# sandyz1000/face-landmark-detector

Hardware: AMD Instinct MI355X
Metric: faces/sec (whole node), 256x256 batch inference: fused preprocess + FCN-8 forward + softmax + top-4 landmark decode + similarity/alignment warp (higher is better)
Workload: dtype f32; 1 GPU; BASELINE configs[1]: batch=64/GPU 256x256x3 uint8 crops, fcn_8(68) vanilla encoder fp32, random-init weights (seed 2), decode top-4 thresh 0, align to 256x256; global_batch=64, parallelism=dp1

## Files before the change

### face-landmark-detector_amd/build.py

```python
from __future__ import annotations

import concurrent.futures
import hashlib
import os
import shutil
import subprocess
import sys

HERE = os.path.dirname(os.path.abspath(__file__))
ROOT = os.path.dirname(HERE)
CSRC = os.path.join(HERE, "csrc")
INCLUDE = os.path.join(ROOT, "include")
OBJ_DIR = os.path.join(HERE, "csrc", "build")
LIB_PATH = os.path.join(HERE, "libflm_hip.so")

SOURCES = [
    "flm_api.hip",
    "flm_pack.hip",
    "flm_enc1.hip",
    "flm_igemm.hip",
    "flm_igemm_bf16.hip",
    "flm_conv3_halo.hip",
    "flm_score1x1.hip",
    "flm_tail_bf16.hip",
    "flm_convt.hip",
    "flm_up3_wreg.hip",
    "flm_decode.hip",
    "flm_decode_stats.hip",
    "flm_cand.hip",
    "flm_misc.hip",
    "flm_frames.hip",
    "flm_warp_fmt.hip",
    "flm_frames_nv12.hip",
    "flm_mesh.hip",
    "flm_track.hip",
    "flm_track_assoc.hip",
    "flm_quality.hip",
    "flm_track_exit.hip",
    "flm_track_views.hip",
    "flm_pose.hip",
    "flm_annotate.hip",
    "flm_flow.hip",
    "flm_mobile.hip",
]
FLAGS = ["--offload-arch=gfx950", "-O3", "-fPIC", "-std=c++17", "-ffp-contract=off",
         "-Wall", "-Wno-unused-function", "-I", INCLUDE, "-I", CSRC]


FILE_FLAGS = {"flm_enc1.hip": ["-mllvm", "-amdgpu-mfma-vgpr-form"]}


def _hipcc() -> str:
    for c in (shutil.which("hipcc"), "/opt/rocm/bin/hipcc"):
        if c and os.path.exists(c):
            return c
    raise RuntimeError("hipcc not found: the HIP extension cannot be built")


def _stamp(paths) -> str:
    h = hashlib.sha256()
    h.update(" ".join(FLAGS).encode())
    h.update(repr(sorted(FILE_FLAGS.items())).encode())
    for p in sorted(paths):
        with open(p, "rb") as f:
            h.update(p.encode())
            h.update(f.read())
    return h.hexdigest()


def build(force: bool = False, verbose: bool = True, extra_flags=()) -> str:
    os.makedirs(OBJ_DIR, exist_ok=True)
    headers = [os.path.join(CSRC, f) for f in os.listdir(CSRC) if f.endswith(".h")] + \
              [os.path.join(INCLUDE, f) for f in os.listdir(INCLUDE) if f.endswith(".h")]
    srcs = [os.path.join(CSRC, s) for s in SOURCES]
    stamp = _stamp(srcs + headers) + " ".join(extra_flags)
    stamp_file = os.path.join(OBJ_DIR, "stamp.txt")
    if not force and os.path.exists(LIB_PATH) and os.path.exists(stamp_file) and open(stamp_file).read() == stamp:
        return LIB_PATH
    hipcc = _hipcc()

    def compile_one(src):
        obj = os.path.join(OBJ_DIR, os.path.basename(src) + ".o")
        cmd = [hipcc, *FLAGS, *FILE_FLAGS.get(os.path.basename(src), []), *extra_flags, "-c", src, "-o", obj]
        r = subprocess.run(cmd, capture_output=True, text=True)
        if r.returncode != 0:
            raise RuntimeError("hipcc failed on %s:\n%s\n%s" % (src, r.stdout, r.stderr))
        if verbose and r.stderr.strip():
            sys.stderr.write(r.stderr)
        return obj

    with concurrent.futures.ThreadPoolExecutor(max_workers=min(8, len(srcs))) as ex:
        objs = list(ex.map(compile_one, srcs))
    cmd = [hipcc, "--offload-arch=gfx950", "-shared", "-fPIC", "-o", LIB_PATH, *objs]
    r = subprocess.run(cmd, capture_output=True, text=True)
    if r.returncode != 0:
        raise RuntimeError("link failed:\n%s\n%s" % (r.stdout, r.stderr))
    with open(stamp_file, "w") as f:
        f.write(stamp)
    if verbose:
        print("built", LIB_PATH)
    return LIB_PATH


if __name__ == "__main__":
    build(force="--force" in sys.argv)
```

### face-landmark-detector_amd/csrc/flm_api.hip

```cpp
#include <cmath>
#include <cstdarg>
#include <cstdio>
#include <cstring>

#include "flm_annotate_dev.h"
#include "flm_common.h"

namespace flm {

static thread_local char g_err[512] = "";

void set_error(const char* fmt, ...) {
  va_list ap;
  va_start(ap, fmt);
  vsnprintf(g_err, sizeof(g_err), fmt, ap);
  va_end(ap);
}

int hip_fail(hipError_t e, const char* what) {
  set_error("HIP error %d (%s) at %s", (int)e, hipGetErrorString(e), what);
  return FLM_ERR_HIP;
}

struct Knob {
  const char* key;
  std::atomic<int> value;
  bool (*valid)(int);
  const char* domain;
};
static Knob g_knobs[] = {
    {"bf16_big_tiles", {1}, nullptr, nullptr},
    {"bf16_lds_dma", {1}, nullptr, nullptr},
    {"bf16_mfma16", {1}, nullptr, nullptr},
    {"bf16_halo_mfma16", {1}, nullptr, nullptr},
    {"f32_two_level", {1}, nullptr, nullptr},
    {"f32_lean_tile", {1}, nullptr, nullptr},
    {"bf16_group_n", {0}, [](int v) { return v >= 0 && v <= 32 && !(v & (v - 1)); }, "0 or a power of two <= 32"},
    {"bf16_conv3_halo", {1}, nullptr, nullptr},
    {"bf16_score1x1", {1}, nullptr, nullptr},
    {"bf16_fused_tail", {1}, nullptr, nullptr},
    {"decode_lds_dma", {1}, nullptr, nullptr},
    {"posmajor_order", {1}, nullptr, nullptr},
    {"warp_rows", {1}, [](int v) { return v == 0 || v == 1 || v == 4; }, "0, 1 or 4"},
    {"up3_cand8", {1}, [](int v) { return v >= 0 && v <= 7; }, "in [0,7]"},
    {"up3_cand8_rows", {0}, [](int v) { return v >= 0 && v <= 8 && !(v & (v - 1)); }, "0, 1, 2, 4 or 8"},
    {"up3_wreg", {0}, [](int v) { return v == 0 || v == 1; }, "0 or 1"},
    {"f32_fc6_rows", {0}, [](int v) { return v == 0 || v == 64 || v == 128; }, "0, 64 or 128"},
};
static_assert(sizeof(g_knobs) / sizeof(g_knobs[0]) == KNOB_COUNT, "one row per KnobId");
int tuning(KnobId id) { return g_knobs[id].value.load(std::memory_order_relaxed); }
static Knob* find_knob(const char* who, const char* key) {
  for (Knob& k : g_knobs)
    if (!strcmp(k.key, key)) return &k;
  set_error("%s: unknown key '%s'", who, key);
  return nullptr;
}

struct ProfRec {
  const char* name;
  hipEvent_t a, b;
};
static ProfRec* g_prof = nullptr;
static int g_prof_cap = 0, g_prof_n = 0;
static char g_prof_filter[32] = "";

struct ProfScope {
  hipStream_t s;
  ProfRec* r;
  ProfScope(hipStream_t st, const char* name) : s(st), r(nullptr) {
    if (name && g_prof && g_prof_n < g_prof_cap && (!g_prof_filter[0] || !strcmp(g_prof_filter, name))) {
      r = &g_prof[g_prof_n++];
      r->name = name;
      (void)hipEventRecord(r->a, s);
    }
  }
  ~ProfScope() {
    if (r) (void)hipEventRecord(r->b, s);
  }
};

struct CandOpts {
  int enable, sub, cap_div;
};
static bool resolve_opts(const flm_forward_opts* o, CandOpts* c) {
  c->enable = 1;
  c->sub = 0;
  c->cap_div = 1;
  if (!o) return true;
  if (o->struct_size < sizeof(flm_forward_opts)) {
    set_error("flm_forward_opts: struct_size %u is smaller than this library's %zu (initialise with flm_forward_opts_init)",
              o->struct_size, sizeof(flm_forward_opts));
    return false;
  }
  if (o->candidate_sub_phases < 0 || o->candidate_sub_phases > 16 || o->candidate_cap_div < 1) {
    set_error("flm_forward_opts: candidate_sub_phases must be in [0,16] and candidate_cap_div >= 1");
    return false;
  }
  c->enable = o->landmark_candidates != 0;
  c->sub = o->candidate_sub_phases;
  c->cap_div = o->candidate_cap_div;
  return true;
}
static int cand_sub_for(const CandOpts& c, int n_points, bool bf16) {
  if (c.sub > 0) return c.sub;
  return n_points <= 8 ? (bf16 ? 4 : 2) : (n_points <= 15 ? 6 : 8);
}
static bool landmark_candidates_enabled(const CandOpts& c, const ConvTGeom& g, int fcn32, int decode_mode, int n_points,
                                        int oh, int ow) {
  return c.enable && !fcn32 && decode_mode == FLM_DECODE_TOPN && n_points >= 1 && n_points <= 32 &&
         convt_candidates_supported(g) && (long long)oh * ow < (1 << 17);
}

struct EncNames {
  char s[kMaxEnc][8];
  EncNames() {
    for (int i = 0; i < kMaxEnc; ++i) snprintf(s[i], sizeof(s[i]), "enc%d", i + 1);
  }
};

static size_t take(size_t& cur, size_t bytes) {
  size_t o = cur;
  cur = align_up(cur + bytes, 256);
  return o;
}

Fcn8Ws fcn8_ws_layout(int n, int h, int w, int C, int dtype, int out_mode, int decode_mode, int n_points,
                      int arch, const flm_forward_opts* opts) {
  Fcn8Ws W;
  CandOpts co;
  if (!resolve_opts(opts, &co)) {
    W = Fcn8Ws();
    W.total = 0;
    return W;
  }
  const ConvTGeom g = convt_geom(C, dtype);
  const ArchSpec A = arch_spec(arch);
  const size_t es = dtype == FLM_BF16 ? 2 : 4;
  size_t cur = 0;
  int hs[kMaxEnc], wsz[kMaxEnc];
  enc_dims(A, h, w, hs, wsz);
  for (int i = 0; i < A.n_enc; ++i) W.act[i] = take(cur, es * (size_t)n * hs[i] * wsz[i] * A.enc[i].cout);
  for (int k = 0; k < 5; ++k) W.f[k] = W.act[A.f_idx[k]];
  const int h5 = h / 32, w5 = w / 32, h4 = h / 16, w4 = w / 16, h3 = h / 8, w3 = w / 8;
  W.fc6 = take(cur, es * (size_t)n * h5 * w5 * kFc);
  W.fc7 = take(cur, es * (size_t)n * h5 * w5 * kFc);
  W.score5 = take(cur, sizeof(float) * (size_t)n * h5 * w5 * g.Cp);
  W.fuse4 = take(cur, sizeof(float) * (size_t)n * h4 * w4 * g.Cp);
  W.seg = take(cur, sizeof(float) * (size_t)n * h3 * w3 * g.Cp);
  W.splitk_bytes = sizeof(float) * 8 * (size_t)n * h5 * w5 * g.Cp;
  {
    const size_t rows = (size_t)n * h5 * w5 < 256 ? (size_t)n * h5 * w5 : 256;
    const size_t fc_bytes = sizeof(float) * 8 * rows * kFc;
    if (fc_bytes > W.splitk_bytes) W.splitk_bytes = fc_bytes;
  }
  if (n <= 4) {
    const size_t enc3_bytes = sizeof(float) * 4 * (size_t)4 * (h / 4) * (w / 4) * 256;
    if (enc3_bytes > W.splitk_bytes) W.splitk_bytes = enc3_bytes;
  }
  W.splitk = take(cur, W.splitk_bytes);
  W.oh = h + (A.fcn32 ? 32 : 8);
  W.ow = w + (A.fcn32 ? 32 : 8);
  W.probs = SIZE_MAX;
  W.decode = SIZE_MAX;
  W.sub = W.tau = W.cand = W.cand_cnt = SIZE_MAX;
  W.cand_cap = W.cand_sub = 0;
  const int stats = out_mode == FLM_OUT_LANDMARKS_STATS;
  if (out_mode == FLM_OUT_LANDMARKS || stats) {
    W.probs = take(cur, sizeof(float) * (size_t)n * W.oh * W.ow * C);
    W.decode = take(cur, decode_ws_bytes(n, W.oh, W.ow, C, decode_mode, n_points, stats));
    if (landmark_candidates_enabled(co, g, A.fcn32, decode_mode, n_points, W.oh, W.ow)) {
      W.cand_sub = cand_sub_for(co, n_points, g.bf16 != 0);
      W.sub = take(cur, sizeof(unsigned) * (size_t)n * convt_sample_slots(g, h3, w3, W.cand_sub) * 16 * g.MT);
      W.tau = take(cur, sizeof(float) * (size_t)n * C);
      W.cand_cap = (int)align_up((size_t)C * 64 * n_points * 4 / co.cap_div, 64);
      if (W.cand_cap < 64) W.cand_cap = 64;
      W.cand = take(cur, sizeof(unsigned long long) * (size_t)n * W.cand_cap);
      W.cand_cnt = take(cur, sizeof(unsigned) * ((size_t)n + 1));
    }
  }
  W.total = cur;
  return W;
}

static int check_dtype_classes(const char* what, int dtype, int C) {
  if (dtype != FLM_F32 && dtype != FLM_BF16) {
    set_error("%s: unknown dtype %d (FLM_F32 = 0, FLM_BF16 = 1)", what, dtype);
    return FLM_ERR_UNSUPPORTED;
  }
  if (C < 1 || C > kMaxClasses) {
    set_error("%s: n_classes must be in [1,%d] (got %d)", what, kMaxClasses, C);
    return FLM_ERR_SHAPE;
  }
  return FLM_OK;
}

static int check_fcn8_shape(int n, int h, int w, int C, int dtype) {
  const int rc = check_dtype_classes("fcn8", dtype, C);
  if (rc) return rc;
  if (n <= 0 || h <= 0 || w <= 0 || (h % 32) || (w % 32)) {
    set_error("fcn8: input must be [N>0, H, W, 3] with H and W multiples of 32 (got n=%d h=%d w=%d)", n, h, w);
// ... 2059 lines not shown
```

### face-landmark-detector_amd/csrc/flm_common.h

```cpp
#pragma once

#include <hip/hip_runtime.h>
#include <stddef.h>
#include <stdint.h>

#include <atomic>
#include <mutex>

#include "flm.h"

namespace flm {

void set_error(const char* fmt, ...);
int hip_fail(hipError_t e, const char* what);

#define FLM_HIP(call)                                            \
  do {                                                           \
    hipError_t e_ = (call);                                      \
    if (e_ != hipSuccess) return ::flm::hip_fail(e_, #call);     \
  } while (0)

#define FLM_LAUNCH_CHECK(what)                                   \
  do {                                                           \
    hipError_t e_ = hipGetLastError();                           \
    if (e_ != hipSuccess) return ::flm::hip_fail(e_, what);      \
  } while (0)

struct FuncAttrOnce {
  std::atomic<unsigned> done{0};
  std::mutex mu;
};
#define FLM_FUNC_ATTR_ONCE(flag, kernel, lds_bytes)                                                        \
  do {                                                                                                     \
    int dev_ = 0;                                                                                          \
    FLM_HIP(hipGetDevice(&dev_));                                                                          \
    const unsigned bit_ = 1u << (dev_ & 31);                                                               \
    if (!((flag).done.load(std::memory_order_acquire) & bit_)) {                                           \
      std::lock_guard<std::mutex> lock_((flag).mu);                                                        \
      if (!((flag).done.load(std::memory_order_relaxed) & bit_)) {                                         \
        FLM_HIP(hipFuncSetAttribute(reinterpret_cast<const void*>(kernel),                                 \
                                    hipFuncAttributeMaxDynamicSharedMemorySize, (int)(lds_bytes)));        \
        (flag).done.fetch_or(bit_, std::memory_order_release);                                             \
      }                                                                                                    \
    }                                                                                                      \
  } while (0)

static inline int cdiv(int a, int b) { return (a + b - 1) / b; }
static inline size_t align_up(size_t x, size_t a) { return (x + a - 1) / a * a; }

constexpr float kBnEps = 1e-3f;

constexpr int kFc = 4096;
constexpr int kMaxClasses = 96;
constexpr int kMaxEnc = 64;

enum EncKind {
  ENC_FIRST3 = 0,
  ENC_CONV3 = 1,
  ENC_MB_CONV1 = 2,
  ENC_MB_DW = 3,
  ENC_MB_PW = 4,
  ENC_RN_CONV1 = 5,
  ENC_MAXPOOL3 = 6,
  ENC_CONV = 7
};
struct EncLayer {
  int cin, cout, bn, pool;
  int kind, stride;
  int k, relu;
  int src, res;
};
struct ArchSpec {
  int n_enc;
  EncLayer enc[kMaxEnc];
  int f_idx[5];
  int fcn32;
  int valid;
};
void enc_dims(const ArchSpec& A, int h, int w, int* hs, int* ws);
inline int enc_has_params(const EncLayer& e) { return e.kind != ENC_MAXPOOL3; }
ArchSpec arch_spec(int arch);

struct ConvTGeom {
  int C;
  int Cp;
  int MT;
  int G;
  int bf16;
};
ConvTGeom convt_geom(int C, int dtype);

struct ConvPack {
  size_t w;
  size_t scale;
  size_t shift;
  int cin, cout, coutpad, kh, kw, pad;
};

struct Fcn8Pack {
  size_t enc1_w;
  size_t enc1_scale, enc1_shift;
  ConvPack enc[kMaxEnc];
  ConvPack fc6, fc7, score5, score4, score3;
  size_t up5, up4, up3;
  ConvTGeom g;
  int dtype;
  int arch;
  ArchSpec spec;
  size_t total;
};
Fcn8Pack fcn8_pack_layout(int C, int dtype, int arch = 0);

struct Fcn8Ws {
  size_t act[kMaxEnc];
  size_t f[5];
  size_t fc6, fc7, score5, fuse4, seg;
  size_t splitk;
  size_t splitk_bytes;
  size_t probs;
  size_t decode;
  size_t sub, tau, cand, cand_cnt;
  int cand_cap;
  int cand_sub;
  size_t total;
  int oh, ow;
};
Fcn8Ws fcn8_ws_layout(int n, int h, int w, int C, int dtype, int out_mode, int decode_mode, int n_points,
                      int arch = 0, const flm_forward_opts* opts = nullptr);

enum KnobId {
  KNOB_BF16_BIG_TILES, KNOB_BF16_LDS_DMA, KNOB_BF16_MFMA16, KNOB_BF16_HALO_MFMA16, KNOB_F32_TWO_LEVEL, KNOB_F32_LEAN_TILE,
  KNOB_BF16_GROUP_N, KNOB_BF16_CONV3_HALO, KNOB_BF16_SCORE1X1, KNOB_BF16_FUSED_TAIL, KNOB_DECODE_LDS_DMA,
  KNOB_POSMAJOR_ORDER, KNOB_WARP_ROWS, KNOB_UP3_CAND8, KNOB_UP3_CAND8_ROWS, KNOB_UP3_WREG, KNOB_F32_FC6_ROWS,
  KNOB_COUNT
};
int tuning(KnobId id);

int launch_pack_fcn(hipStream_t s, const flm_fcn_params& p, int C, const Fcn8Pack& L, char* blob);

int launch_enc1(hipStream_t s, const void* x, int in_format, int n, int h, int w, const float* w1p,
                const float* scale, const float* shift, void* f1, int out_bf16, int pool);

struct IgemmDesc {
  const void* x;
  const void* wt;
  const float* scale;
  const float* shift;
  void* y;
  int bf16;
  int out_f32;
  int n, h, w, cin;
  int cout;
  int coutpad;
  int ldc;
  int kh, kw, pad;
  int relu, pool, posmajor;
  int stride;
  const void* res;
  float* splitk_ws;
  size_t splitk_ws_bytes;
};
int launch_igemm(hipStream_t s, const IgemmDesc& d);
int igemm_occupancy(size_t lds_bytes);
int igemm_posmajor_rows_last();
int launch_seg_fused_bf16(hipStream_t s, const float* fuse4, const void* w4_packed, const void* f3, const void* w3,
                          const float* scale3, const float* shift3, float* seg, int n, int h4, int w4d, int C, int Cp,
                          int G, int cin3, int coutpad3);

struct ConvTDesc {
  const float* x;
  const void* wf;
  const float* skip;
  void* y;
  int n, hi, wi;
  int ho, wo;
  int s;
  int ldy;
  int epilogue;
  ConvTGeom g;
  int sub = 0;
  const float* tau = nullptr;
  unsigned long long* cand = nullptr;
  unsigned* cand_cnt = nullptr;
  int cand_cap = 0;
  const unsigned* gate = nullptr;
  void* scratch = nullptr;
  size_t scratch_bytes = 0;
};
int launch_convt(hipStream_t s, const ConvTDesc& d);
int convt_candidates_supported(const ConvTGeom& g);
__host__ __device__ inline int convt_share_layout(const ConvTGeom& g, int s) {
  return g.C == 68 && (g.bf16 ? g.G == 9 : g.G == 17) && (s % 4) == 0;
}
int convt_sample_slots(const ConvTGeom& g, int hi, int wi, int sub);
int launch_cand_tau(hipStream_t s, const unsigned* wave_max, int n, int slots, int ld, int l, int n_points, float* tau);

int launch_mb_conv1(hipStream_t s, const void* x, int in_format, int n, int h, int w, const float* wgt,
                    const float* scale, const float* shift, void* y, int bf16);
int launch_mb_depthwise(hipStream_t s, const void* x, int n, int h, int w, int c, int stride, const float* wgt,
                        const float* scale, const float* shift, void* y, int bf16);
int launch_rn_conv1(hipStream_t s, const void* x, int in_format, int n, int h, int w, const float* wgt,
                    const float* scale, const float* shift, void* y, int bf16);
int launch_maxpool3(hipStream_t s, const void* x, int n, int h, int w, int c, void* y, int bf16);

size_t decode_ws_bytes(int n, int h, int w, int l, int mode, int n_points, int stats = 0);
int launch_decode(hipStream_t s, const float* hm, int n, int h, int w, int l, int mode, int n_points, float thresh,
                  double* out, void* ws, size_t ws_bytes, const unsigned* gate = nullptr, int stats = 0);
size_t decode_sweep_ws_bytes(int n, int h, int w, int l, const int* modes, int n_modes);
int launch_decode_sweep(hipStream_t s, const float* hm, int n, int h, int w, int l, const int* modes, int n_modes,
                        float thresh, double* out, void* ws, size_t ws_bytes);
int launch_gaussian_heatmaps(hipStream_t s, const double* kp, int n, int l, int h, int w, double two_sigma_sq,
                             float* out);
int launch_cand_merge(hipStream_t s, const unsigned long long* cand, unsigned* cand_cnt, int n, int w, int l,
                      int n_points, float thresh, int cap, double* out, int stats = 0);

int launch_preprocess(hipStream_t s, const uint8_t* img, int n, int h, int w, int norm, float* out);
int launch_similarity(hipStream_t s, const double* lm, const double* tmpl, int n, int k, double sx, double sy, float* m);
int launch_similarity_weighted(hipStream_t s, const double* lm, size_t lm_stride, const double* wt, size_t w_stride,
                               const double* tmpl, int n, int k, double sx, double sy, float* m);
int launch_warp(hipStream_t s, const void* src, int src_is_u8, int n, int hs, int ws, const float* m, float* dst,
                int hd, int wd);
int launch_crop_resize(hipStream_t s, const uint8_t* frame, int fh, int fw, const int32_t* boxes, int k,
                       uint8_t* out, int oh, int ow, const int32_t* frame_idx = nullptr, size_t frame_stride = 0,
                       int nframes = 0);
int launch_landmarks_to_frame(hipStream_t s, const double* lm, const int32_t* boxes, int k, int c, int grid_h,
                              int grid_w, int fh, int fw, double* out);
int launch_warp_frames(hipStream_t s, const uint8_t* frames, size_t frame_stride, int nframes, int fh, int fw,
                       const int32_t* frame_idx, const int32_t* boxes, const float* m, int k, float* dst, int hd,
                       int wd, int samples);
int launch_warp_fmt(hipStream_t s, const void* src, int src_is_u8, int n, int hs, int ws, const float* m, void* dst, int hd,
                    int wd, const flm_image_format* fmt);
int launch_warp_frames_fmt(hipStream_t s, const uint8_t* frames, size_t frame_stride, int nframes, int fh, int fw,
                           const int32_t* frame_idx, const int32_t* boxes, const float* m, int k, void* dst, int hd,
                           int wd, int samples, const flm_image_format* fmt);

int bgr_ring_check(const char* who, size_t frame_stride, int nframes, int fh, int fw);

int launch_frames_to_bgr_nv12(hipStream_t s, const uint8_t* frames, size_t frame_stride, int nframes, int fh, int fw,
                              const flm_frame_format* src, uint8_t* out);
int launch_crop_resize_nv12(hipStream_t s, const uint8_t* frames, size_t frame_stride, int nframes, int fh, int fw,
                            const int32_t* boxes, const int32_t* frame_idx, int k, uint8_t* out, int oh, int ow,
                            const flm_frame_format* src);
int launch_warp_frames_nv12(hipStream_t s, const uint8_t* frames, size_t frame_stride, int nframes, int fh, int fw,
                            const int32_t* frame_idx, const int32_t* boxes, const float* m, int k, void* dst, int hd,
                            int wd, int samples, const flm_image_format* fmt, const flm_frame_format* src);
size_t nv12_format_bytes(const char* who, const flm_frame_format* src, int fh, int fw);
struct Nv12Geom;
int nv12_ring_geometry(const char* who, const flm_frame_format* src, size_t frame_stride, int nframes, int fh, int fw,
                       Nv12Geom* g);

int launch_mesh_map(hipStream_t s, const double* pts, const int32_t* tris, int p, int t, int hd, int wd, uint8_t* map);
int launch_mesh_affines(hipStream_t s, const double* lm, int lm_stride, const float* m, const double* pts,
                        const int32_t* tris, int p, int a, int t, int k, double min_det, float* aff);
int launch_warp_mesh_frames(hipStream_t s, const uint8_t* frames, size_t frame_stride, int nframes, int fh, int fw,
                            const int32_t* frame_idx, const int32_t* boxes, const double* lm, int lm_stride,
                            const float* m, const double* pts, const int32_t* tris, int p, int a, int t,
                            const uint8_t* map, int k, void* dst, int hd, int wd, int samples,
                            const flm_image_format* fmt, const flm_frame_format* src, double min_det, float* aff_out);

int launch_track_seed(hipStream_t s, const int32_t* boxes, int k, int in_h, int in_w, int fh, int fw, float* m,
                      int32_t* status);
int launch_landmarks_from_crop(hipStream_t s, const double* lm, size_t lm_stride, const float* m, int k, int c, double sx,
                               double sy, double* out);
int launch_track_step(hipStream_t s, const char* who, const double* lm, size_t lm_stride, const double* wt, size_t w_stride,
                      const float* m_crop, const int32_t* boxes, int k, int c, double sx, double sy, int in_h, int in_w,
                      int fh, int fw, const double* tmpl_crop, const double* tmpl_align, const flm_track_opts* opts,
                      double* lm_frame, float* m_align, float* m_next, int32_t* boxes_next, int32_t* status,
                      const flm_track_filter* filt , double dt, double* state, double* lm_raw,
                      const int32_t* slot , int n_slots,
                      const double* dt_rows, int32_t* status_rows);
int launch_track_gather_streams(hipStream_t s, const int32_t* active, int a, int n_streams, int k,
                                const int32_t* frame_idx_stream, const double* dt_stream, const float* m_crop,
                                const int32_t* boxes, const double* best_q, int32_t* reset, int32_t* slot_c, float* m_c,
                                int32_t* boxes_c, int32_t* frame_idx_c, double* dt_c, double* best_q_c, int32_t* reset_c);
struct TrackLiveArgs {
  const int32_t* boxes;
  const float* m_crop;
  int s, k, fh, fw, n;
  const int32_t* stream_on;
  const int32_t* frame_idx_stream;
  const double* dt_stream;
  double dt;
  const double* best_q;
  int32_t* reset;
  double* age;
  int32_t* cursor;
// ... 139 lines not shown
```

### face-landmark-detector_amd/csrc/flm_igemm.hip

```cpp
#include <type_traits>
#include <vector>

#include "flm_igemm_args.h"

#ifndef FLM_IGEMM_VAR
#define FLM_IGEMM_VAR 0
#endif

namespace flm {

typedef float f32x16 __attribute__((ext_vector_type(16)));
typedef __bf16 bf16x8 __attribute__((ext_vector_type(8)));

constexpr int BM = 128, BN = 128, BK = 32;
constexpr int TILE_F = BM * BK;

__device__ __forceinline__ int swz(int row, int chunk) { return row * BK + ((chunk ^ ((row >> 1) & 7)) << 2); }

__device__ __forceinline__ float f4c(const float4& v, int i) { return i == 0 ? v.x : (i == 1 ? v.y : (i == 2 ? v.z : v.w)); }

template <bool BF, int IDX, bool HALF = false>
__device__ __forceinline__ void mfma_slot(const float4& a0, const float4& a1, const float4& b0, const float4& b1,
                                          f32x16& c00, f32x16& c01, f32x16& c10, f32x16& c11) {
  if constexpr (BF) {
// ... 745 lines not shown
  if (hipGetDevice(&dev) != hipSuccess) return 128;
  std::lock_guard<std::mutex> lock(g_rows_mu);
  for (const RowsEntry& c : g_rows_cache)
    if (c.h == a.h && c.w == a.w && c.kh == a.kh && c.kw == a.kw && c.pad == a.pad && c.n == a.n && c.ntiles == a.ntiles && c.dev == dev)
      return c.rows;
  int cus = 0, occ128 = 0, occ64 = 0;
  if (hipDeviceGetAttribute(&cus, hipDeviceAttributeMultiprocessorCount, dev) != hipSuccess ||
      hipOccupancyMaxActiveBlocksPerMultiprocessor(&occ128, reinterpret_cast<const void*>(&igemm_kernel<false, 2, true, true, false, BM>),
                                                   256, igemm_lds_bytes<BM>()) != hipSuccess ||
      hipOccupancyMaxActiveBlocksPerMultiprocessor(&occ64, reinterpret_cast<const void*>(&igemm_kernel<false, 2, true, true, false, 64>),
                                                   256, igemm_lds_bytes<64>()) != hipSuccess)
    return 128;
  const int rows = posmajor_pick_rows(a, cus / 8 * occ128, cus / 8 * occ64);
  if (g_rows_cache.size() < 256) g_rows_cache.push_back({a.h, a.w, a.kh, a.kw, a.pad, a.n, a.ntiles, dev, rows});
  return rows;
}

template <bool BF, bool TWO = false>
static int dispatch(hipStream_t s, const IgemmDesc& d, const IgemmArgs& a) {
  if constexpr (TWO) {
    if (d.posmajor) {
      const int rows = posmajor_rows_for(a);
      g_rows_last.store(rows, std::memory_order_relaxed);
      if (rows == 64) return d.relu ? launch_t<BF, 2, true, TWO, false, 64>(s, a) : launch_t<BF, 2, false, TWO, false, 64>(s, a);
    }
  }
  if constexpr (TWO) {
    if (!d.posmajor && tuning(KNOB_F32_LEAN_TILE)) {
      if (d.pool) return d.relu ? launch_t<BF, 1, true, TWO, true>(s, a) : launch_t<BF, 1, false, TWO, true>(s, a);
      return d.relu ? launch_t<BF, 0, true, TWO, true>(s, a) : launch_t<BF, 0, false, TWO, true>(s, a);
    }
  }
  if (d.pool) return d.relu ? launch_t<BF, 1, true, TWO>(s, a) : launch_t<BF, 1, false, TWO>(s, a);
  if (d.posmajor) return d.relu ? launch_t<BF, 2, true, TWO>(s, a) : launch_t<BF, 2, false, TWO>(s, a);
  return d.relu ? launch_t<BF, 0, true, TWO>(s, a) : launch_t<BF, 0, false, TWO>(s, a);
}


int launch_igemm(hipStream_t s, const IgemmDesc& d) {
  const int es = d.bf16 ? 2 : 4;
  const int bke = 128 / es;
  if (d.cin % bke != 0 || d.coutpad % BN != 0 || d.cout > d.coutpad || d.kh * d.kw > 64) {
    set_error("igemm: unsupported shape cin=%d coutpad=%d cout=%d k=%dx%d (%s)", d.cin, d.coutpad, d.cout, d.kh, d.kw,
              d.bf16 ? "bf16" : "fp32");
    return FLM_ERR_SHAPE;
  }
  if (d.pool && ((d.h & 1) || (d.w & 1))) {
    set_error("igemm: pooled layer needs even h,w (got %dx%d)", d.h, d.w);
    return FLM_ERR_SHAPE;
  }
  const int stride = d.stride > 0 ? d.stride : 1;
  const int ho = (d.h + 2 * d.pad - d.kh) / stride + 1, wo = (d.w + 2 * d.pad - d.kw) / stride + 1;
  if ((stride != 1 || d.res) && (d.pool || d.posmajor)) {
    set_error("igemm: stride / residual are only built for the row-major pixel order");
    return FLM_ERR_UNSUPPORTED;
  }
  if (stride == 1 && (ho != d.h || wo != d.w)) {
    set_error("igemm: stride-1 layers must be 'same' (k=%dx%d pad=%d)", d.kh, d.kw, d.pad);
    return FLM_ERR_SHAPE;
  }
  const long long M = (long long)d.n * ho * wo;
  if (M <= 0 || M > (1ll << 30)) {
    set_error("igemm: pixel count %lld out of range", M);
    return FLM_ERR_SHAPE;
  }
  if ((long long)d.n * d.h * d.w * d.cin * es >= (1ll << 32) || (long long)d.coutpad * d.kh * d.kw * d.cin >= (1ll << 31)) {
    set_error("igemm: tensor exceeds the 32-bit offset range (split the batch)");
    return FLM_ERR_SHAPE;
  }
  IgemmArgs a;
  a.x = d.x; a.wt = d.wt; a.scale = d.scale; a.shift = d.shift; a.y = d.y;
  a.out_f32 = d.bf16 ? d.out_f32 : 1;
  a.relu_max = d.relu == 2 ? 6.0f : 3.402823466e38f;
  a.n = d.n; a.h = d.h; a.w = d.w; a.cin = d.cin; a.cout = d.cout; a.ldc = d.ldc;
  a.ho = ho; a.wo = wo; a.stride = stride; a.res = d.res;
  a.kh = d.kh; a.kw = d.kw; a.pad = d.pad;
  a.M = (int)M;
  a.K = d.kh * d.kw * d.cin;
  a.mtiles = cdiv(a.M, BM);
  a.cpt = d.cin / bke;
  a.kw_magic = (65536 + d.kw - 1) / d.kw;
  a.ksplit = 1;
  a.gm = a.gn = 1;
  a.grp_magic = 0;
  a.posperm_on = 0;
  for (int k = 0; k < 8; ++k) a.posperm[k] = 0ull;
  a.dx = a.dy = 1;
  a.dx_magic = a.dy_magic = 1u << 30;
  a.dx_shift = a.dy_shift = 0;
  a.all_taps = 0;
  a.part = nullptr;
  const int tiles = cdiv(a.M, BM) * cdiv(d.cout, BN);
  const int faces = d.n > 0 ? d.n : 1;
  const bool few_faces = d.kh * d.kw > 1 && d.cout < 1024 && faces <= 4 && tiles <= 64 * faces;
  const bool narrow_1x1 = !d.bf16 && d.kh * d.kw == 1 && d.cin / bke >= 32 && d.cout <= BN;
  const int tile_cap = narrow_1x1 ? 0x7fffffff : ((d.cout >= 1024 || few_faces) ? 256 : 64);
  if (d.splitk_ws && !d.res && stride == 1 && tiles <= tile_cap && (!d.pool || (a.M & 3) == 0) &&
      (d.kh * d.kw == 1 ? a.cpt >= 32 : (a.cpt >= 4 && (d.cout >= 1024 || tiles <= 16 * faces || few_faces))) &&
      (d.relu != 2 || d.pool)) {
    int ks = (tiles <= 64 || narrow_1x1) ? 8 : (tiles <= 128 ? 4 : 2);
    if (few_faces && tiles > 16 * faces) ks = 8;
    int per = d.kh * d.kw == 1 ? 8 : 1;
    if (d.kh * d.kw == 1 && tiles <= 8) {
      ks = 32;
      per = 4;
    }
    if (d.kh * d.kw > 1) {
      if (ks > d.kh * d.kw * a.cpt / 8) ks = d.kh * d.kw * a.cpt / 8;
    } else if (ks > a.cpt / per) {
      ks = a.cpt / per;
    }
    const size_t part_rows = few_faces ? (size_t)(a.M / faces) * 4 : (size_t)a.M;
    if (ks > 1 && (size_t)ks * part_rows * d.ldc * sizeof(float) <= d.splitk_ws_bytes) {
      a.ksplit = ks;
      a.part = d.splitk_ws;
    }
  }
  a.ntiles = cdiv(d.cout, BN);
  if (d.bf16) {
    const int sk = launch_score1x1_bf16(s, a, d.relu, d.pool, d.posmajor, d.coutpad);
    if (sk < 0) return sk;
    if (sk == 1) return FLM_OK;
    const int halo = launch_conv3_halo_bf16(s, a, d.relu, d.pool, d.posmajor);
    if (halo < 0) return halo;
    if (halo == 1) return FLM_OK;
    const int big = launch_igemm_bf16_big(s, a, d.relu, d.pool, d.posmajor, d.coutpad);
    if (big < 0) return big;
    if (big == 1) return FLM_OK;
  }
  int rc;
  const int two_level = tuning(KNOB_F32_TWO_LEVEL);
  if (d.bf16) {
    rc = dispatch<true>(s, d, a);
  } else if (!two_level) {
    rc = dispatch<false>(s, d, a);
  } else {
    const int dense = d.kh * d.kw * a.cpt;
    if (dense >= 8192) {
      set_error("igemm: %d k-steps per output exceed the group divider's range", dense);
      return FLM_ERR_SHAPE;
    }
    int grp = 2;
    while ((grp + 1) * (grp + 1) <= dense) ++grp;
    a.grp_magic = (65536 + grp - 1) / grp;
    const long long face_in = (long long)d.h * d.w * d.cin * 4,
                    face_out = (long long)(d.pool ? (ho / 2) * (wo / 2) : ho * wo) * d.ldc * 4;
    const long long lim = (1ll << 31) - (1ll << 22);
    if (face_in >= lim) {
      set_error("igemm: one face exceeds the 2 GiB buffer range of the fp32 kernel");
      return FLM_ERR_SHAPE;
    }
    const int max_faces = (int)(lim / face_in);
    if (d.n <= max_faces) {
      rc = dispatch<false, true>(s, d, a);
    } else {
      if (a.ksplit > 1) {
        set_error("igemm: batch slicing is not built for split-K layers");
        return FLM_ERR_UNSUPPORTED;
      }
      rc = FLM_OK;
      for (int f0 = 0; f0 < d.n && rc == FLM_OK; f0 += max_faces) {
        IgemmArgs b = a;
        b.n = d.n - f0 < max_faces ? d.n - f0 : max_faces;
        b.x = reinterpret_cast<const char*>(a.x) + (size_t)f0 * face_in;
        b.y = reinterpret_cast<char*>(a.y) + (size_t)f0 * face_out;
        if (a.res) b.res = reinterpret_cast<const char*>(a.res) + (size_t)f0 * face_out;
        b.M = b.n * ho * wo;
        b.mtiles = cdiv(b.M, BM);
        rc = dispatch<false, true>(s, d, b);
      }
    }
  }
  if (rc || a.ksplit <= 1) return rc;
  const size_t total = (size_t)a.M * d.ldc;
  const int blocks = (int)((total + 255) / 256 < 2048 ? (total + 255) / 256 : 2048);
  if (d.pool) {
    splitk_reduce_pool_kernel<<<blocks, 256, 0, s>>>(a.part, a.scale, a.shift, a.y, a.M, d.ldc, d.cout, a.ksplit, d.relu,
                                                     a.relu_max, d.bf16 && !d.out_f32);
    FLM_LAUNCH_CHECK("splitk_reduce_pool_kernel");
    return FLM_OK;
  }
  splitk_reduce_kernel<<<blocks, 256, 0, s>>>(a.part, a.scale, a.shift, a.y, a.M, d.ldc, d.cout, a.ksplit, d.relu,
                                              d.bf16 && !d.out_f32);
  FLM_LAUNCH_CHECK("splitk_reduce_kernel");
  return FLM_OK;
}

}
```

### face-landmark-detector_amd/csrc/flm_igemm_args.h

```cpp
#pragma once
#include <algorithm>
#include <vector>

#include "flm_common.h"

namespace flm {

struct IgemmArgs {
  const void* x;
  const void* wt;
  const float* scale;
  const float* shift;
  void* y;
  int out_f32;
  float relu_max;
  int n, h, w, cin;
  int ho, wo, stride;
  const void* res;
  int cout, ldc;
  int kh, kw, pad;
  int M;
  int K;
  int mtiles, ntiles;
  int cpt;
// ... 85 lines not shown
  if (n >= 32) {
    int nn = nn0 + (m - m_first), pos = pos0;
    if (nn >= n) {
      nn -= n;
      pos = pos1;
    }
    return (size_t)nn * hw + pos;
  }
  return (size_t)(m % n) * hw + m / n;
}

struct PospermEntry {
  int h, w, kh, kw, pad, g, on;
  unsigned long long table[8];
};
bool posperm_cache_get(PospermEntry& e);
void posperm_cache_put(const PospermEntry& e);

inline void posmajor_fill_perm(IgemmArgs& a, int bm) {
  a.posperm_on = 0;
  for (int k = 0; k < 8; ++k) a.posperm[k] = 0ull;
  const int P = a.h * a.w;
  if (!tuning(KNOB_POSMAJOR_ORDER) || P > 64 || P < 2 || a.n < 32 || a.n >= bm || bm % a.n != 0 || a.kh * a.kw > 64) return;
  const int g = bm / a.n;
  PospermEntry ent = {a.h, a.w, a.kh, a.kw, a.pad, g, 0, {0, 0, 0, 0, 0, 0, 0, 0}};
  if (!posperm_cache_get(ent)) {
    unsigned long long mask[64];
    long long key[3][64];
    for (int p = 0; p < P; ++p) {
      const int y = p / a.w, x = p % a.w;
      const int kx_lo = a.pad - x > 0 ? a.pad - x : 0, kx_hi = a.pad + a.w - 1 - x < a.kw - 1 ? a.pad + a.w - 1 - x : a.kw - 1;
      const int ky_lo = a.pad - y > 0 ? a.pad - y : 0, ky_hi = a.pad + a.h - 1 - y < a.kh - 1 ? a.pad + a.h - 1 - y : a.kh - 1;
      unsigned long long m = 0ull;
      for (int ky = ky_lo; ky <= ky_hi; ++ky)
        for (int kx = kx_lo; kx <= kx_hi; ++kx) m |= 1ull << (ky * a.kw + kx);
      mask[p] = m;
      key[0][p] = ((((long long)ky_lo * 64 + ky_hi) * 64 + kx_lo) * 64 + kx_hi) * 64 + p;
      key[1][p] = ((long long)((y + 1) / 2) * 64 + (x + 1) / 2) * 64 + p;
      key[2][p] = (long long)(64 - __builtin_popcountll(m)) * (1ll << 40) + key[0][p];
    }
    long long best_cost = -1;
    int best[64];
    for (int start = 0; start < 3; ++start) {
      int order[64];
      for (int p = 0; p < P; ++p) order[p] = p;
      for (int i = 1; i < P; ++i)
        for (int j = i; j > 0 && key[start][order[j]] < key[start][order[j - 1]]; --j) {
          const int t = order[j]; order[j] = order[j - 1]; order[j - 1] = t;
        }
      auto group_cost = [&](int gi) {
        unsigned long long u = 0ull;
        int rows = 0;
        for (int i = gi * g; i < (gi + 1) * g && i < P; ++i) { u |= mask[order[i]]; ++rows; }
        return (long long)__builtin_popcountll(u) * rows;
      };
      for (int sweep = 0; sweep < 64; ++sweep) {
        bool better = false;
        for (int i = 0; i < P; ++i)
          for (int j = i + 1; j < P; ++j) {
            if (i / g == j / g) continue;
            const long long before = group_cost(i / g) + group_cost(j / g);
            int t = order[i]; order[i] = order[j]; order[j] = t;
            if (group_cost(i / g) + group_cost(j / g) < before) { better = true; continue; }
            t = order[i]; order[i] = order[j]; order[j] = t;
          }
        if (!better) break;
      }
      long long cost = 0;
      for (int gi = 0; gi * g < P; ++gi) cost += group_cost(gi);
      if (best_cost < 0 || cost < best_cost) {
        best_cost = cost;
        for (int p = 0; p < P; ++p) best[p] = order[p];
      }
    }
    bool identity = true;
    for (int i = 0; i < P; ++i) {
      identity = identity && best[i] == i;
      ent.table[i >> 3] |= (unsigned long long)best[i] << ((i & 7) * 8);
    }
    ent.on = identity ? 0 : 1;
    posperm_cache_put(ent);
  }
  a.posperm_on = ent.on;
  for (int k = 0; k < 8; ++k) a.posperm[k] = ent.table[k];
}


inline unsigned long long posmajor_tile_mask(const IgemmArgs& a, int bm, int t) {
  const int m_lo = t * bm, m_hi = (m_lo + bm < a.M ? m_lo + bm : a.M) - 1;
  unsigned long long mask = 0ull;
  for (int p = m_lo / a.n; p <= m_hi / a.n; ++p) mask |= posmajor_posmask(posmajor_pos(a, p), a.h, a.w, a.kh, a.kw, a.pad);
  return mask;
}

inline long long posmajor_makespan(IgemmArgs a, int bm, int slots_per_xcd) {
  a.mtiles = (a.M + bm - 1) / bm;
  posmajor_fill_perm(a, bm);
  std::vector<int> wk((size_t)a.mtiles);
  for (int t = 0; t < a.mtiles; ++t) wk[(size_t)t] = __builtin_popcountll(posmajor_tile_mask(a, bm, t)) * (bm / 64);
  std::sort(wk.begin(), wk.end(), [](int x, int y) { return x > y; });
  const bool by_xcd = (a.ntiles & 7) == 0;
  const int copies = by_xcd ? a.ntiles >> 3 : 1, rounds = by_xcd ? 1 : a.ntiles;
  std::vector<long long> load((size_t)(by_xcd ? slots_per_xcd : 8 * slots_per_xcd), 0ll);
  for (int round = 0; round < rounds; ++round)
    for (int t = 0; t < a.mtiles; ++t)
      for (int c = 0; c < copies; ++c) *std::min_element(load.begin(), load.end()) += wk[(size_t)t];
  return *std::max_element(load.begin(), load.end());
}

constexpr int kRows64SurchargePermille = 0;
constexpr int kRows64MaxTiles = 2048;

inline int posmajor_pick_rows(const IgemmArgs& a, int slots128_per_xcd, int slots64_per_xcd) {
  if (a.ksplit > 1 || a.n >= 128 || (a.M + 63) / 64 > kRows64MaxTiles || slots128_per_xcd < 1 || slots64_per_xcd < 1) return 128;
  const long long m128 = posmajor_makespan(a, 128, slots128_per_xcd) * slots128_per_xcd,
                  m64 = posmajor_makespan(a, 64, slots64_per_xcd) * slots64_per_xcd;
  return m64 * (1000 + kRows64SurchargePermille) < m128 * 1000 ? 64 : 128;
}

__device__ __forceinline__ unsigned short f2bf(float v) { return __builtin_bit_cast(unsigned short, (__bf16)v); }

__device__ __forceinline__ uint2 quad_transpose_bf16(float r0, float r1, float r2, float r3, int q) {
  typedef float f32x2_t __attribute__((ext_vector_type(2)));
  typedef __bf16 bf16x2_t __attribute__((ext_vector_type(2)));
  const unsigned p01 = __builtin_bit_cast(unsigned, __builtin_convertvector((f32x2_t){r0, r1}, bf16x2_t));
  const unsigned p23 = __builtin_bit_cast(unsigned, __builtin_convertvector((f32x2_t){r2, r3}, bf16x2_t));
  const unsigned o01 = (unsigned)__builtin_amdgcn_mov_dpp((int)p01, 0xB1, 0xf, 0xf, true);
  const unsigned o23 = (unsigned)__builtin_amdgcn_mov_dpp((int)p23, 0xB1, 0xf, 0xf, true);
  const unsigned sel = (q & 1) ? 0x03020706u : 0x05040100u;
  const unsigned t01 = __builtin_amdgcn_perm(o01, p01, sel);
  const unsigned t23 = __builtin_amdgcn_perm(o23, p23, sel);
  const bool low = q < 2;
  const unsigned recv = (unsigned)__builtin_amdgcn_mov_dpp((int)(low ? t23 : t01), 0x4E, 0xf, 0xf, true);
  return make_uint2(low ? t01 : recv, low ? recv : t23);
}

constexpr unsigned kOobOffset = 0x80000000u;
constexpr int kSrdFlags = 0x00020000;

typedef int dma_srd __attribute__((ext_vector_type(4)));
__device__ __forceinline__ dma_srd dma_make_srd(const void* base) {
  const unsigned long long b = reinterpret_cast<unsigned long long>(base);
  return (dma_srd){(int)(unsigned)b, (int)(unsigned)((b >> 32) & 0xffffu), 0x7fffffff, kSrdFlags};
}
__device__ __forceinline__ void dma_load16(dma_srd srd, unsigned lds_addr, unsigned voffset, int soffset) {
  asm volatile("s_nop 0\n\tbuffer_load_dwordx4 %0, %1, %2 offen lds"
               :
               : "v"(voffset), "s"(srd), "s"(soffset), "{m0}"(lds_addr)
               : "memory");
}

int launch_igemm_bf16_big(hipStream_t s, const IgemmArgs& a, int relu, int pool, int posmajor, int coutpad);
int launch_score1x1_bf16(hipStream_t s, const IgemmArgs& a, int relu, int pool, int posmajor, int coutpad);
int launch_conv3_halo_bf16(hipStream_t s, const IgemmArgs& a, int relu, int pool, int posmajor);

}
```

Baseline: 7871 faces/s.

## Add streaming fp32 MFMA kernel for 1x1 score convolutions with register-held weights

Adds a dedicated fp32 kernel for 1x1 score convolutions with 256 input channels and at most 96 outputs. Each wave keeps its weight slice in registers, the kernel runs as a persistent grid of twice the CU count, and 32-row activation blocks are double-buffered into LDS via buffer-load-to-LDS DMA before feeding 32x32x2 f32 MFMAs. The goal is to replace the general implicit-GEMM tiles, which waste most of their N dimension on narrow-output layers. Accumulation is split across grouped partial sums, and the grp_magic check is meant to keep the summation order matching the original kernel. It is enabled by default through a new knob.

```diff
diff --git a/face-landmark-detector_amd/build.py b/face-landmark-detector_amd/build.py
--- a/face-landmark-detector_amd/build.py
+++ b/face-landmark-detector_amd/build.py
@@ -22,6 +22,7 @@
     "flm_igemm_bf16.hip",
     "flm_conv3_halo.hip",
     "flm_score1x1.hip",
+    "flm_score1x1_f32.hip",
     "flm_tail_bf16.hip",
     "flm_convt.hip",
     "flm_up3_wreg.hip",
diff --git a/face-landmark-detector_amd/csrc/flm_api.hip b/face-landmark-detector_amd/csrc/flm_api.hip
--- a/face-landmark-detector_amd/csrc/flm_api.hip
+++ b/face-landmark-detector_amd/csrc/flm_api.hip
@@ -46,6 +46,7 @@
     {"up3_cand8_rows", {0}, [](int v) { return v >= 0 && v <= 8 && !(v & (v - 1)); }, "0, 1, 2, 4 or 8"},
     {"up3_wreg", {0}, [](int v) { return v == 0 || v == 1; }, "0 or 1"},
     {"f32_fc6_rows", {0}, [](int v) { return v == 0 || v == 64 || v == 128; }, "0, 64 or 128"},
+    {"f32_score_stream", {1}, nullptr, nullptr},
 };
 static_assert(sizeof(g_knobs) / sizeof(g_knobs[0]) == KNOB_COUNT, "one row per KnobId");
 int tuning(KnobId id) { return g_knobs[id].value.load(std::memory_order_relaxed); }
diff --git a/face-landmark-detector_amd/csrc/flm_common.h b/face-landmark-detector_amd/csrc/flm_common.h
--- a/face-landmark-detector_amd/csrc/flm_common.h
+++ b/face-landmark-detector_amd/csrc/flm_common.h
@@ -132,6 +132,7 @@
   KNOB_BF16_BIG_TILES, KNOB_BF16_LDS_DMA, KNOB_BF16_MFMA16, KNOB_BF16_HALO_MFMA16, KNOB_F32_TWO_LEVEL, KNOB_F32_LEAN_TILE,
   KNOB_BF16_GROUP_N, KNOB_BF16_CONV3_HALO, KNOB_BF16_SCORE1X1, KNOB_BF16_FUSED_TAIL, KNOB_DECODE_LDS_DMA,
   KNOB_POSMAJOR_ORDER, KNOB_WARP_ROWS, KNOB_UP3_CAND8, KNOB_UP3_CAND8_ROWS, KNOB_UP3_WREG, KNOB_F32_FC6_ROWS,
+  KNOB_F32_SCORE_STREAM,
   KNOB_COUNT
 };
 int tuning(KnobId id);
diff --git a/face-landmark-detector_amd/csrc/flm_igemm.hip b/face-landmark-detector_amd/csrc/flm_igemm.hip
--- a/face-landmark-detector_amd/csrc/flm_igemm.hip
+++ b/face-landmark-detector_amd/csrc/flm_igemm.hip
@@ -921,6 +921,9 @@
     }
     const int max_faces = (int)(lim / face_in);
     if (d.n <= max_faces) {
+      const int sk = launch_score1x1_f32(s, a, d.relu, d.pool, d.posmajor, d.coutpad);
+      if (sk < 0) return sk;
+      if (sk == 1) return FLM_OK;
       rc = dispatch<false, true>(s, d, a);
     } else {
       if (a.ksplit > 1) {
diff --git a/face-landmark-detector_amd/csrc/flm_igemm_args.h b/face-landmark-detector_amd/csrc/flm_igemm_args.h
--- a/face-landmark-detector_amd/csrc/flm_igemm_args.h
+++ b/face-landmark-detector_amd/csrc/flm_igemm_args.h
@@ -261,6 +261,7 @@
 
 int launch_igemm_bf16_big(hipStream_t s, const IgemmArgs& a, int relu, int pool, int posmajor, int coutpad);
 int launch_score1x1_bf16(hipStream_t s, const IgemmArgs& a, int relu, int pool, int posmajor, int coutpad);
+int launch_score1x1_f32(hipStream_t s, const IgemmArgs& a, int relu, int pool, int posmajor, int coutpad);
 int launch_conv3_halo_bf16(hipStream_t s, const IgemmArgs& a, int relu, int pool, int posmajor);
 
 }
diff --git a/face-landmark-detector_amd/csrc/flm_score1x1_f32.hip b/face-landmark-detector_amd/csrc/flm_score1x1_f32.hip
--- /dev/null
+++ b/face-landmark-detector_amd/csrc/flm_score1x1_f32.hip
@@ -0,0 +1,161 @@
+#include <atomic>
+
+#include "flm_igemm_args.h"
+
+namespace flm {
+
+typedef float f32x16_sf __attribute__((ext_vector_type(16)));
+
+constexpr int SF_K = 256, SF_STEPS = SF_K / 32;
+constexpr int SF_GRP = 2;
+constexpr int SF_ROWS = 32;
+constexpr int SF_STAGE = SF_ROWS * 128;
+constexpr int SF_BLOCK = SF_STEPS * SF_STAGE;
+
+struct ScoreF32Args {
+  const float* x;
+  const float* wt;
+  const float* scale;
+  const float* shift;
+  float* y;
+  int M, cout, ldc;
+  int nblocks;
+  int relu;
+  float relu_max;
+};
+
+template <int NT>
+__global__ __launch_bounds__(64 * NT) __attribute__((amdgpu_waves_per_eu(1, 2))) void score1x1_f32_kernel(ScoreF32Args a) {
+  __shared__ __attribute__((aligned(16))) char sf_smem[2 * SF_BLOCK];
+  typedef __attribute__((address_space(3))) char lds_char;
+  const int lane = threadIdx.x & 63;
+  const int wave = __builtin_amdgcn_readfirstlane(threadIdx.x >> 6);
+  const int lr = lane & 31, lh = lane >> 5;
+
+  float4 bw[SF_STEPS][4];
+  {
+    const float* wrow = a.wt + (size_t)(32 * wave + lr) * SF_K + 4 * lh;
+#pragma unroll
+    for (int s = 0; s < SF_STEPS; ++s)
+#pragma unroll
+      for (int t = 0; t < 4; ++t) bw[s][t] = *reinterpret_cast<const float4*>(wrow + 32 * s + 8 * t);
+  }
+  const int col = 32 * wave + lr;
+  const bool cok = col < a.cout;
+  const float sc = a.scale[col], sh = a.shift[col];
+  const unsigned lane_off = (unsigned)(4 * lh) * (unsigned)a.ldc + (unsigned)col;
+
+  const unsigned lds0 = (unsigned)(size_t)((lds_char*)sf_smem);
+  const int r8 = lane >> 3, pc = lane & 7;
+  const unsigned rowoff0 = (unsigned)(r8 * SF_K * 4 + ((pc ^ (r8 >> 1)) << 4));
+  auto request_block = [&](int b, int buf) {
+    const int m0 = b * SF_ROWS;
+    const dma_srd xdma = dma_make_srd(reinterpret_cast<const char*>(a.x) + (size_t)m0 * SF_K * 4);
+    const int left = a.M - m0 - r8;
+    for (int r = wave; r < 4 * SF_STEPS; r += NT) {
+      const int s = r >> 2, q = r & 3;
+      const unsigned vo = 8 * q < left ? (rowoff0 ^ ((unsigned)(q & 1) << 6)) + (unsigned)q * (8 * SF_K * 4) : kOobOffset;
+      dma_load16(xdma, lds0 + buf * SF_BLOCK + s * SF_STAGE + q * 1024, vo, s * 128);
+    }
+  };
+
+  const int fa0 = lr * 128 + ((lh ^ ((lr >> 1) & 7)) << 4);
+
+  f32x16_sf zero16;
+#pragma unroll
+  for (int r = 0; r < 16; ++r) zero16[r] = 0.f;
+
+  int buf = 0;
+  if ((int)blockIdx.x < a.nblocks) request_block(blockIdx.x, 0);
+  for (int b = blockIdx.x; b < a.nblocks; b += gridDim.x) {
+    __builtin_amdgcn_s_waitcnt(0x0f70);
+    __syncthreads();
+    if (b + (int)gridDim.x < a.nblocks) request_block(b + gridDim.x, buf ^ 1);
+
+    const char* ab = sf_smem + buf * SF_BLOCK;
+    f32x16_sf acc = zero16, sum = zero16, top = zero16;
+    float4 af = *reinterpret_cast<const float4*>(ab + fa0), an = af;
+#pragma unroll
+    for (int s = 0; s < SF_STEPS; ++s) {
+#pragma unroll
+      for (int t = 0; t < 4; ++t) {
+        if (t < 3) an = *reinterpret_cast<const float4*>(ab + s * SF_STAGE + (fa0 ^ ((t + 1) << 5)));
+        else if (s + 1 < SF_STEPS) an = *reinterpret_cast<const float4*>(ab + (s + 1) * SF_STAGE + fa0);
+        if (t == 0) {
+          sum += acc;
+          asm volatile("" : "+v"(sum));
+          acc = __builtin_amdgcn_mfma_f32_32x32x2f32(af.x, bw[s][0].x, zero16, 0, 0, 0);
+        } else {
+          acc = __builtin_amdgcn_mfma_f32_32x32x2f32(af.x, bw[s][t].x, acc, 0, 0, 0);
+        }
+        acc = __builtin_amdgcn_mfma_f32_32x32x2f32(af.y, bw[s][t].y, acc, 0, 0, 0);
+        acc = __builtin_amdgcn_mfma_f32_32x32x2f32(af.z, bw[s][t].z, acc, 0, 0, 0);
+        acc = __builtin_amdgcn_mfma_f32_32x32x2f32(af.w, bw[s][t].w, acc, 0, 0, 0);
+        af = an;
+        __builtin_amdgcn_sched_barrier(0);
+      }
+      if (s > 0 && s % SF_GRP == 0) {
+        top += sum;
+        asm volatile("" : "+v"(top));
+        sum = zero16;
+      }
+    }
+    acc = top + (sum + acc);
+
+    if (cok) {
+      float* yt = a.y + (size_t)b * SF_ROWS * a.ldc;
+      const int lim = a.M - b * SF_ROWS - 4 * lh;
+#pragma unroll
+      for (int r = 0; r < 16; ++r) {
+        const int rc = (r & 3) + 8 * (r >> 2);
+        float u = fmaf(acc[r], sc, sh);
+        if (a.relu) u = fminf(fmaxf(u, 0.f), a.relu_max);
+        if (rc < lim) (yt + (unsigned)rc * (unsigned)a.ldc)[lane_off] = u;
+      }
+    }
+    buf ^= 1;
+  }
+}
+
+static int sf_cu_count() {
+  static std::atomic<int> cache[32];
+  int dev = 0;
+  if (hipGetDevice(&dev) != hipSuccess) return -1;
+  const int slot = dev & 31;
+  int cus = cache[slot].load(std::memory_order_relaxed);
+  if (cus > 0) return cus;
+  if (hipDeviceGetAttribute(&cus, hipDeviceAttributeMultiprocessorCount, dev) != hipSuccess || cus < 1) return -1;
+  cache[slot].store(cus, std::memory_order_relaxed);
+  return cus;
+}
+
+template <int NT>
+static int launch_sf(hipStream_t s, const ScoreF32Args& k, int grid) {
+  score1x1_f32_kernel<NT><<<grid, 64 * NT, 0, s>>>(k);
+  FLM_LAUNCH_CHECK("score1x1_f32_kernel");
+  return 1;
+}
+
+int launch_score1x1_f32(hipStream_t s, const IgemmArgs& a, int relu, int pool, int posmajor, int coutpad) {
+  if (!tuning(KNOB_F32_SCORE_STREAM) || a.kh != 1 || a.kw != 1 || a.pad != 0 || a.stride != 1 || a.res || pool || posmajor ||
+      a.ksplit > 1 || a.cout < 1 || a.cout > 96 || a.cout > a.ldc || coutpad < 32 * cdiv(a.cout, 32) || a.cin != SF_K ||
+      a.M < 1 || a.grp_magic != (65536 + SF_GRP - 1) / SF_GRP)
+    return 0;
+  const int cus = sf_cu_count();
+  if (cus < 1) return hip_fail(hipErrorInvalidDevice, "score1x1_f32: compute unit count");
+  ScoreF32Args k;
+  k.x = static_cast<const float*>(a.x);
+  k.wt = static_cast<const float*>(a.wt);
+  k.scale = a.scale;
+  k.shift = a.shift;
+  k.y = static_cast<float*>(a.y);
+  k.M = a.M; k.cout = a.cout; k.ldc = a.ldc;
+  k.nblocks = cdiv(a.M, SF_ROWS);
+  k.relu = relu != 0;
+  k.relu_max = a.relu_max;
+  const int grid = k.nblocks < 2 * cus ? k.nblocks : 2 * cus;
+  const int nt = cdiv(a.cout, 32);
+  return nt == 1 ? launch_sf<1>(s, k, grid) : (nt == 2 ? launch_sf<2>(s, k, grid) : launch_sf<3>(s, k, grid));
+}
+
+}
```

Result: no change. 7866 faces/s (-0.1%).
